# heiheishuang/MuDG

Hardware: AMD Instinct MI355X
Metric: DDIM denoise steps/sec, MDM1024 576x1024x16f (CFG: 2 UNet forwards + fused update per step, per clip) (higher is better)
Workload: dtype bf16; 1 GPU; MDM1024 latents (B=1,4,16,72,128) + c_concat 8ch, context (B,333,1024), 50-step uniform_trailing DDIM schedule, cfg 7.5, guidance_rescale 0.7, eta 1.0, v-prediction, dynamic rescale; clips_per_gpu=1, parallelism=clip-DP x1 (no in-step collective), launch=hipGraph replay of each UNet pass (cond+uncond batched)

## Files before the change

### mudg_amd/csrc/attention.hip

```cpp
#include "common.h"
#include <cstdlib>
#include <type_traits>

namespace {

constexpr int QB = 128;
constexpr int KB = 64;
constexpr int ALD = 72;
constexpr int ATILE = 64 * ALD;

template <bool TWO>
__global__ __launch_bounds__(256, 2) void attn_kernel(const MudgAttnDesc p, const int nqt, const int total) {
    __shared__ __attribute__((aligned(16))) h16 Ks[2 * ATILE];
    __shared__ __attribute__((aligned(16))) h16 Vs[2 * ATILE];

    const int tid = threadIdx.x, lane = tid & 63, wave = tid >> 6;
    const int l31 = lane & 31, hi = lane >> 5;

    int w;
    {
        const int q8 = total >> 3, r8 = total & 7;
        const int xcd = blockIdx.x & 7, idx = blockIdx.x >> 3;
        w = (xcd < r8 ? xcd * (q8 + 1) : r8 * (q8 + 1) + (xcd - r8) * q8) + idx;
    }
// ... 394 lines not shown
    u32x4 kr[2], vr[2];
    auto load_tiles = [&](int kt) {
        const int j0 = kt * KB;
#pragma unroll
        for (int i = 0; i < 2; ++i) {
            const int row = lrow + 32 * i;
            const int j = j0 + row;
            kr[i] = (j < p.Nk) ? ld16(Kp + (int64_t)j * p.ldk + kc * 8) : zero16();
            const int jc = j0 + kc * 8;
            u32x4 v = zero16();
            if (jc < p.Nk) {
                v = ld16(Vp + (int64_t)row * p.ldvt + jc);
                if (jc + 8 > p.Nk) {
                    h16x8 hv = as_h16x8(v);
#pragma unroll
                    for (int e = 0; e < 8; ++e) if (jc + e >= p.Nk) hv[e] = (h16)0.f;
                    v = as_u32x4(hv);
                }
            }
            vr[i] = v;
        }
    };
    const int vlo = (kc >> 1) * 16 + ((kc & 1) ? 4 : 0), vhi = (kc >> 1) * 16 + ((kc & 1) ? 12 : 8);
    auto stage = [&](int buf) {
#pragma unroll
        for (int i = 0; i < 2; ++i) {
            st16(&Ks[buf * ATILE + (lrow + 32 * i) * ALD + kc * 8], kr[i]);
            h16* vrow = &Vs[buf * ATILE + (lrow + 32 * i) * ALD];
            *reinterpret_cast<u32x2*>(vrow + vlo) = u32x2{vr[i][0], vr[i][1]};
            *reinterpret_cast<u32x2*>(vrow + vhi) = u32x2{vr[i][2], vr[i][3]};
        }
    };

    f32x16 o[2][2];
#pragma unroll
    for (int qb = 0; qb < 2; ++qb)
#pragma unroll
        for (int r = 0; r < 16; ++r) { o[qb][0][r] = 0.f; o[qb][1][r] = 0.f; }
    float m_run[2] = {-INFINITY, -INFINITY}, l_run[2] = {0.f, 0.f};
    const float c = p.q_prescaled ? 1.0f : p.scale * 1.4426950408889634f;

    const int nkt = (p.Nk + KB - 1) / KB;
    load_tiles(0);
    stage(0);
    __syncthreads();

    for (int kt = 0; kt < nkt; ++kt) {
        const int cur = kt & 1;
        const bool more = kt + 1 < nkt;
        if (more) load_tiles(kt + 1);

        f32x16 s[2][2];
#pragma unroll
        for (int sub = 0; sub < 2; ++sub) {
#pragma unroll
            for (int qb = 0; qb < 2; ++qb)
#pragma unroll
                for (int r = 0; r < 16; ++r) s[qb][sub][r] = 0.f;
            const h16* kp = Ks + cur * ATILE + (sub * 32 + l31) * ALD + hi * 8;
#pragma unroll
            for (int ks = 0; ks < 4; ++ks) {
                const h16x8 kf = *reinterpret_cast<const h16x8*>(kp + ks * 16);
                s[0][sub] = MFMA_32x32x16(kf, qf[0][ks], s[0][sub]);
                s[1][sub] = MFMA_32x32x16(kf, qf[1][ks], s[1][sub]);
            }
        }
        if (kt * KB + KB > p.Nk) {
#pragma unroll
            for (int sub = 0; sub < 2; ++sub)
#pragma unroll
                for (int r = 0; r < 16; ++r) {
                    const int j = kt * KB + sub * 32 + (r & 3) + 8 * (r >> 2) + 4 * hi;
                    if (j >= p.Nk) { s[0][sub][r] = -INFINITY; s[1][sub][r] = -INFINITY; }
                }
        }

        h16x8 pk[2][2][2];
#pragma unroll
        for (int qb = 0; qb < 2; ++qb) {
            float mx = s[qb][0][0];
#pragma unroll
            for (int r = 1; r < 16; ++r) mx = fmaxf(mx, s[qb][0][r]);
#pragma unroll
            for (int r = 0; r < 16; ++r) mx = fmaxf(mx, s[qb][1][r]);
            mx = fmaxf(mx, __shfl_xor(mx, 32, 64));
            const bool grew = !__all(mx <= m_run[qb]);
            const float m_new = grew ? fmaxf(m_run[qb], mx) : m_run[qb];
            const float alpha = grew ? __builtin_amdgcn_exp2f((m_run[qb] - m_new) * c) : 1.0f;
            const float mc = m_new * c;
            m_run[qb] = m_new;
            float ps = 0.f;
#pragma unroll
            for (int sub = 0; sub < 2; ++sub)
#pragma unroll
                for (int r = 0; r < 16; ++r) {
                    const float e = __builtin_amdgcn_exp2f(fmaf(s[qb][sub][r], c, -mc));
                    ps += e;
                    pk[qb][sub][r >> 3][r & 7] = (h16)e;
                }
            l_run[qb] = l_run[qb] * alpha + ps;
            if (grew) {
#pragma unroll
                for (int r = 0; r < 16; ++r) { o[qb][0][r] *= alpha; o[qb][1][r] *= alpha; }
            }
        }

#pragma unroll
        for (int dt = 0; dt < 2; ++dt) {
            const h16* vp = Vs + cur * ATILE + (dt * 32 + l31) * ALD + 8 * hi;
#pragma unroll
            for (int sub = 0; sub < 2; ++sub)
#pragma unroll
                for (int jj = 0; jj < 2; ++jj) {
                    const h16x8 vf = *reinterpret_cast<const h16x8*>(vp + sub * 32 + jj * 16);
                    o[0][dt] = MFMA_32x32x16(vf, pk[0][sub][jj], o[0][dt]);
                    o[1][dt] = MFMA_32x32x16(vf, pk[1][sub][jj], o[1][dt]);
                }
        }

        if (more) stage(cur ^ 1);
        __syncthreads();
    }

#pragma unroll
    for (int qb = 0; qb < 2; ++qb) {
        const float l_tot = l_run[qb] + __shfl_xor(l_run[qb], 32, 64);
        const float inv = 1.f / l_tot;
        if (p.Lse && qok[qb] && hi == 0) p.Lse[((int64_t)f * p.Nq + qrow[qb]) * p.heads + h] = m_run[qb] * c + __log2f(l_tot);
        if (qok[qb]) {
            h16* orow = Op + (int64_t)qrow[qb] * p.ldo;
#pragma unroll
            for (int dt = 0; dt < 2; ++dt)
#pragma unroll
                for (int g = 0; g < 4; ++g) {
                    h16* dst = orow + dt * 32 + 8 * g + 4 * hi;
                    float v[4];
#pragma unroll
                    for (int j = 0; j < 4; ++j) v[j] = o[qb][dt][4 * g + j] * inv;
                    if (p.accumulate) {
                        Pack8 old; old.u = *reinterpret_cast<const u32x2*>(dst);
#pragma unroll
                        for (int j = 0; j < 4; ++j) v[j] += (float)old.h[j];
                    }
                    Pack8 nw;
#pragma unroll
                    for (int j = 0; j < 4; ++j) nw.h[j] = (h16)v[j];
                    *reinterpret_cast<u32x2*>(dst) = nw.u;
                }
        }
    }
}

constexpr int DTILE = 64 * 64;
#ifdef MUDG_OPERAND_FP16
constexpr float LEAN_LIMIT = 32768.f;
#else
constexpr float LEAN_LIMIT = 1099511627776.f;
#endif

__device__ __forceinline__ __amdgpu_buffer_rsrc_t attn_rsrc(const h16* base) {
    return __builtin_amdgcn_make_buffer_rsrc(const_cast<h16*>(base), 0, (int)0x80000000u, 0x00020000);
}
typedef __attribute__((address_space(3))) void* attn_lptr_t;

typedef __attribute__((ext_vector_type(8))) int i32x8;

template <bool LEAN, bool F8>
__global__ __launch_bounds__(256, 2) void attn64d_kernel(const MudgAttnDesc p, const int nqt, const int total) {
    static_assert(LEAN || !F8, "the fp8 score path builds on the lean softmax");
    __shared__ __attribute__((aligned(1024))) h16 Ks[F8 ? DTILE : 2 * DTILE];
    __shared__ __attribute__((aligned(1024))) h16 Vs[2 * DTILE];

    const int tid = threadIdx.x, lane = tid & 63;
    const int wave = __builtin_amdgcn_readfirstlane(tid >> 6);
    const int l31 = lane & 31, hi = lane >> 5;
    int w;
    {
        const int q8 = total >> 3, r8 = total & 7;
        const int xcd = blockIdx.x & 7, idx = blockIdx.x >> 3;
        w = (xcd < r8 ? xcd * (q8 + 1) : r8 * (q8 + 1) + (xcd - r8) * q8) + idx;
    }
    const int pair = w / nqt, qt = w - pair * nqt;
    const int f = pair / p.heads, h = pair - f * p.heads;
    const int kvb = f / p.kv_div;

    const h16* Qp = reinterpret_cast<const h16*>(p.Q) + (int64_t)f * p.Nq * p.ldq + h * 64;
    const h16* Kp = reinterpret_cast<const h16*>(p.K) + (int64_t)kvb * p.Nk * p.ldk + h * 64;
    const h16* Vp = reinterpret_cast<const h16*>(p.Vt) + (int64_t)kvb * p.svt + (int64_t)(h * 64) * p.ldvt;
    h16* Op = reinterpret_cast<h16*>(p.O) + (int64_t)f * p.Nq * p.ldo + h * 64;

    int qrow[2];
    bool qok[2];
    h16x8 qf[2][F8 ? 1 : 4];
    i32x8 qf8[2];
    int qsc[2] = {127, 127};
    const unsigned char* K8p = nullptr;
    const unsigned char* Ksp = nullptr;
#pragma unroll
    for (int qb = 0; qb < 2; ++qb) {
        qrow[qb] = qt * 256 + wave * 64 + qb * 32 + l31;
        qok[qb] = qrow[qb] < p.Nq;
        if constexpr (F8) {
            const unsigned char* q8 = reinterpret_cast<const unsigned char*>(p.Q8) + ((int64_t)f * p.Nq + qrow[qb]) * p.ldq8 + h * 64 + hi * 16;
            const u32x4 a = qok[qb] ? ld16(q8) : zero16(), b = qok[qb] ? ld16(q8 + 32) : zero16();
            qf8[qb] = i32x8{(int)a[0], (int)a[1], (int)a[2], (int)a[3], (int)b[0], (int)b[1], (int)b[2], (int)b[3]};
            if (qok[qb]) qsc[qb] = reinterpret_cast<const unsigned char*>(p.Qs)[((int64_t)f * p.Nq + qrow[qb]) * p.ldqs + h * 2 + hi];
        } else {
#pragma unroll
            for (int ks = 0; ks < 4; ++ks)
                qf[qb][ks] = as_h16x8(qok[qb] ? ld16(Qp + (int64_t)qrow[qb] * p.ldq + ks * 16 + hi * 8) : zero16());
        }
    }
    if constexpr (F8) {
        K8p = reinterpret_cast<const unsigned char*>(p.K8) + (int64_t)kvb * p.Nk * p.ldk8 + h * 64;
        Ksp = reinterpret_cast<const unsigned char*>(p.Ks) + (int64_t)kvb * p.Nk * p.ldks + h * 2;
    }

    const __amdgpu_buffer_rsrc_t rK = F8 ? __builtin_amdgcn_make_buffer_rsrc(const_cast<unsigned char*>(K8p), 0, (int)0x80000000u, 0x00020000)
                                         : attn_rsrc(Kp);
    const __amdgpu_buffer_rsrc_t rV = attn_rsrc(Vp);
    unsigned vk[2], vv[2];
#pragma unroll
    for (int i = 0; i < 2; ++i) {
        const int row = 16 * wave + 8 * i + (lane >> 3), slot = lane & 7;
        const int chunk = slot ^ ((row >> 1) & 7);
        const int i16 = row & 15;
        const int key = (row & ~15) | (i16 & 3) | ((i16 & 8) >> 1) | ((i16 & 4) << 1);
        vk[i] = (unsigned)key * (unsigned)p.ldk * 2u + (unsigned)chunk * 16u;
        vv[i] = (unsigned)row * (unsigned)p.ldvt * 2u + (unsigned)chunk * 16u;
    }
    int kscale_off[2] = {0, 0};
    if constexpr (F8) {
        const int row = 16 * wave + (lane >> 2), slot = lane & 3;
        const int chunk = slot ^ ((row >> 2) & 3);
        const int i16 = row & 15;
        const int key = (row & ~15) | (i16 & 3) | ((i16 & 8) >> 1) | ((i16 & 4) << 1);
        vk[0] = (unsigned)key * (unsigned)p.ldk8 + (unsigned)chunk * 16u;
#pragma unroll
        for (int sub = 0; sub < 2; ++sub) {
            const int r = sub * 32 + l31, j16 = r & 15;
            const int k = (r & ~15) | (j16 & 3) | ((j16 & 8) >> 1) | ((j16 & 4) << 1);
            kscale_off[sub] = k * p.ldks + hi;
        }
    }
    auto request = [&](int kt, int buf) {
        const int sv = kt * 128;
        if constexpr (F8) {
            unsigned char* ks8 = reinterpret_cast<unsigned char*>(Ks);
            __builtin_amdgcn_raw_ptr_buffer_load_lds(rK, (attn_lptr_t)(ks8 + buf * 4096 + (16 * wave) * 64), 16, (int)vk[0], kt * 64 * p.ldk8, 0, 0);
        }
#pragma unroll
        for (int i = 0; i < 2; ++i) {
            if constexpr (!F8)
                __builtin_amdgcn_raw_ptr_buffer_load_lds(rK, (attn_lptr_t)(Ks + buf * DTILE + (16 * wave + 8 * i) * 64), 16, (int)vk[i], kt * 64 * p.ldk * 2, 0, 0);
            __builtin_amdgcn_raw_ptr_buffer_load_lds(rV, (attn_lptr_t)(Vs + buf * DTILE + (16 * wave + 8 * i) * 64), 16, (int)vv[i], sv, 0, 0);
        }
    };
    const int sw = (l31 >> 1) & 7;
    const int sw8 = (l31 >> 2) & 3;
    auto score_block = [&](int buf, int sub, f32x16& s0, f32x16& s1, int kscale) {
        if constexpr (F8) {
            const unsigned char* kp = reinterpret_cast<const unsigned char*>(Ks) + buf * 4096 + (sub * 32 + l31) * 64;
            const u32x4 a = ld16(kp + ((hi ^ sw8) << 4)), b = ld16(kp + (((2 + hi) ^ sw8) << 4));
            const i32x8 kf = {(int)a[0], (int)a[1], (int)a[2], (int)a[3], (int)b[0], (int)b[1], (int)b[2], (int)b[3]};
            s0 = __builtin_amdgcn_mfma_scale_f32_32x32x64_f8f6f4(kf, qf8[0], s0, 0, 0, 0, kscale, 0, qsc[0]);
            s1 = __builtin_amdgcn_mfma_scale_f32_32x32x64_f8f6f4(kf, qf8[1], s1, 0, 0, 0, kscale, 0, qsc[1]);
        } else {
            const h16* kp = Ks + buf * DTILE + (sub * 32 + l31) * 64;
#pragma unroll
            for (int ks = 0; ks < 4; ++ks) {
                const h16x8 kf = *reinterpret_cast<const h16x8*>(kp + (((ks * 2 + hi) ^ sw) << 3));
                s0 = MFMA_32x32x16(kf, qf[0][ks], s0);
                s1 = MFMA_32x32x16(kf, qf[1][ks], s1);
            }
        }
    };

    f32x16 o[2][2];
    float m_run[2], l_run[2];
    const float c = p.q_prescaled ? 1.0f : p.scale * 1.4426950408889634f;
    const int nkt = p.Nk / KB;
    bool overflow = false;

    auto key_loop = [&](auto lean_tag) {
        constexpr bool LN = decltype(lean_tag)::value;
#pragma unroll
        for (int qb = 0; qb < 2; ++qb) {
#pragma unroll
            for (int r = 0; r < 16; ++r) { o[qb][0][r] = 0.f; o[qb][1][r] = 0.f; }
            m_run[qb] = LN ? 0.f : -INFINITY;
            l_run[qb] = 0.f;
        }
        request(0, 0);
        __syncthreads();
        if constexpr (LN) {
            f32x16 s0[2][2];
#pragma unroll
            for (int sub = 0; sub < 2; ++sub) {
#pragma unroll
                for (int qb = 0; qb < 2; ++qb)
#pragma unroll
                    for (int r = 0; r < 16; ++r) s0[qb][sub][r] = 0.f;
                score_block(0, sub, s0[0][sub], s0[1][sub], F8 ? (int)Ksp[kscale_off[sub]] : 127);
            }
#pragma unroll
            for (int qb = 0; qb < 2; ++qb) {
                float mx = s0[qb][0][0];
#pragma unroll
                for (int r = 1; r < 16; ++r) mx = fmaxf(mx, s0[qb][0][r]);
#pragma unroll
                for (int r = 0; r < 16; ++r) mx = fmaxf(mx, s0[qb][1][r]);
                m_run[qb] = fmaxf(mx, __shfl_xor(mx, 32, 64));
            }
        }

        int ksc[2] = {127, 127};
        if constexpr (F8) { ksc[0] = Ksp[kscale_off[0]]; ksc[1] = Ksp[kscale_off[1]]; }
        for (int kt = 0; kt < nkt; ++kt) {
            const int cur = kt & 1;
            if (kt + 1 < nkt) request(kt + 1, cur ^ 1);
            int ksn[2] = {127, 127};
            if constexpr (F8) {
                if (kt + 1 < nkt) {
                    ksn[0] = Ksp[(int64_t)(kt + 1) * 64 * p.ldks + kscale_off[0]];
                    ksn[1] = Ksp[(int64_t)(kt + 1) * 64 * p.ldks + kscale_off[1]];
                }
            }

            f32x16 s[2][2];
#pragma unroll
            for (int sub = 0; sub < 2; ++sub) {
#pragma unroll
                for (int qb = 0; qb < 2; ++qb) {
                    const float init = LN ? -m_run[qb] : 0.f;
#pragma unroll
                    for (int r = 0; r < 16; ++r) s[qb][sub][r] = init;
                }
                score_block(cur, sub, s[0][sub], s[1][sub], ksc[sub]);
            }
            if constexpr (F8) { ksc[0] = ksn[0]; ksc[1] = ksn[1]; }

            h16x8 pk[2][2][2];
#pragma unroll
            for (int qb = 0; qb < 2; ++qb) {
                if constexpr (LN) {
                    float ps = 0.f;
#pragma unroll
                    for (int sub = 0; sub < 2; ++sub)
#pragma unroll
                        for (int r = 0; r < 16; ++r) {
                            const float e = __builtin_amdgcn_exp2f(s[qb][sub][r]);
                            ps += e;
                            pk[qb][sub][r >> 3][r & 7] = (h16)e;
                        }
                    l_run[qb] += ps;
                    overflow = overflow || !(ps <= LEAN_LIMIT);
                } else {
                    float mx = s[qb][0][0];
#pragma unroll
                    for (int r = 1; r < 16; ++r) mx = fmaxf(mx, s[qb][0][r]);
#pragma unroll
                    for (int r = 0; r < 16; ++r) mx = fmaxf(mx, s[qb][1][r]);
                    mx = fmaxf(mx, __shfl_xor(mx, 32, 64));
                    const bool grew = !__all(mx <= m_run[qb]);
                    const float m_new = grew ? fmaxf(m_run[qb], mx) : m_run[qb];
                    const float alpha = grew ? __builtin_amdgcn_exp2f((m_run[qb] - m_new) * c) : 1.0f;
                    const float mc = m_new * c;
                    m_run[qb] = m_new;
                    float ps = 0.f;
#pragma unroll
                    for (int sub = 0; sub < 2; ++sub)
#pragma unroll
                        for (int r = 0; r < 16; ++r) {
                            const float e = __builtin_amdgcn_exp2f(fmaf(s[qb][sub][r], c, -mc));
                            ps += e;
                            pk[qb][sub][r >> 3][r & 7] = (h16)e;
                        }
                    l_run[qb] = l_run[qb] * alpha + ps;
                    if (grew) {
#pragma unroll
                        for (int r = 0; r < 16; ++r) { o[qb][0][r] *= alpha; o[qb][1][r] *= alpha; }
                    }
                }
            }

#pragma unroll
            for (int dt = 0; dt < 2; ++dt) {
                const h16* vp = Vs + cur * DTILE + (dt * 32 + l31) * 64;
#pragma unroll
                for (int sub = 0; sub < 2; ++sub)
#pragma unroll
                    for (int jj = 0; jj < 2; ++jj) {
                        const h16x8 vf = *reinterpret_cast<const h16x8*>(vp + (((4 * sub + 2 * jj + hi) ^ sw) << 3));
                        o[0][dt] = MFMA_32x32x16(vf, pk[0][sub][jj], o[0][dt]);
                        o[1][dt] = MFMA_32x32x16(vf, pk[1][sub][jj], o[1][dt]);
                    }
            }
            __syncthreads();
        }
    };

    if constexpr (LEAN) {
        key_loop(std::true_type{});
        if (__syncthreads_or(overflow ? 1 : 0)) key_loop(std::false_type{});
    } else {
        key_loop(std::false_type{});
    }

#pragma unroll
    for (int qb = 0; qb < 2; ++qb) {
        const float l_tot = l_run[qb] + __shfl_xor(l_run[qb], 32, 64);
        const float inv = 1.f / l_tot;
        if (p.Lse && qok[qb] && hi == 0) p.Lse[((int64_t)f * p.Nq + qrow[qb]) * p.heads + h] = m_run[qb] * c + __log2f(l_tot);
        if (qok[qb]) {
            h16* orow = Op + (int64_t)qrow[qb] * p.ldo;
#pragma unroll
            for (int dt = 0; dt < 2; ++dt)
#pragma unroll
                for (int g = 0; g < 4; ++g) {
                    h16* dst = orow + dt * 32 + 8 * g + 4 * hi;
                    float v[4];
#pragma unroll
                    for (int j = 0; j < 4; ++j) v[j] = o[qb][dt][4 * g + j] * inv;
                    if (p.accumulate) {
                        Pack8 old; old.u = *reinterpret_cast<const u32x2*>(dst);
#pragma unroll
                        for (int j = 0; j < 4; ++j) v[j] += (float)old.h[j];
                    }
                    Pack8 nw;
#pragma unroll
                    for (int j = 0; j < 4; ++j) nw.h[j] = (h16)v[j];
                    *reinterpret_cast<u32x2*>(dst) = nw.u;
                }
        }
    }
}

constexpr int TATTN_ITEMS = 4;

template <int TP>
__global__ __launch_bounds__(256, TP == 16 ? 3 : 1) void tattn_kernel(const h16* __restrict__ QKV, h16* __restrict__ O,
                                                     int B, int T, int HW, int heads, int ldqkv, int ldo,
                                                     float scale, int total) {
    constexpr int DP = 64 / TP, DW = 64 / DP;
    __shared__ __attribute__((aligned(16))) h16 Ks[4][TP * 64];
    __shared__ __attribute__((aligned(16))) h16 Vs[4][TP * 64];

    const int tid = threadIdx.x, lane = tid & 63, wave = tid >> 6;
    const int tq = lane / DP, dp = lane % DP;
    const int C = heads * 64;
    const int w0 = (blockIdx.x * 4 + wave) * TATTN_ITEMS;

    u32x4 qn[DW / 8], kn[DW / 8], vn[DW / 8];
    int64_t rown = 0; int hn = 0; bool okn = false;
    auto fetch = [&](int w) {
        okn = w < total && tq < T;
        const int bp = w < total ? w / heads : 0;
        hn = w < total ? w - bp * heads : 0;
        const int b = bp / HW, px = bp - b * HW;
        rown = ((int64_t)(b * T + tq) * HW + px);
        const h16* src = QKV + rown * ldqkv + hn * 64 + dp * DW;
#pragma unroll
        for (int i = 0; i < DW / 8; ++i) {
            qn[i] = okn ? ld16(src + i * 8) : zero16();
            kn[i] = okn ? ld16(src + C + i * 8) : zero16();
            vn[i] = okn ? ld16(src + 2 * C + i * 8) : zero16();
        }
    };
    fetch(w0);

    for (int it = 0; it < TATTN_ITEMS; ++it) {
        if (w0 + it >= total) break;
        h16x8 qv[DW / 8];
        const int64_t row = rown; const int h = hn; const bool rok = okn;
        __builtin_amdgcn_wave_barrier();
#pragma unroll
        for (int i = 0; i < DW / 8; ++i) {
            qv[i] = as_h16x8(qn[i]);
            st16(&Ks[wave][tq * 64 + dp * DW + i * 8], kn[i]);
            st16(&Vs[wave][tq * 64 + dp * DW + i * 8], vn[i]);
        }
        __builtin_amdgcn_wave_barrier();
        if (it + 1 < TATTN_ITEMS) fetch(w0 + it + 1);

        float sc[TP];
        float mx = -INFINITY;
#pragma unroll
        for (int j = 0; j < TP; ++j) {
            float a = 0.f;
#pragma unroll
            for (int i = 0; i < DW / 8; ++i) {
                const h16x8 kk = *reinterpret_cast<const h16x8*>(&Ks[wave][j * 64 + dp * DW + i * 8]);
#pragma unroll
                for (int e = 0; e < 8; e += 2) {
                    const h16x2 qp = {qv[i][e], qv[i][e + 1]}, kp = {kk[e], kk[e + 1]};
                    a = DOT2_H16(qp, kp, a);
                }
            }
#pragma unroll
            for (int o = 1; o < DP; o <<= 1) a += __shfl_xor(a, o, 64);
            a = (j < T) ? a * scale : -INFINITY;
            sc[j] = a;
            mx = fmaxf(mx, a);
        }
        float sum = 0.f;
#pragma unroll
        for (int j = 0; j < TP; ++j) { sc[j] = __expf(sc[j] - mx); sum += sc[j]; }
        const float inv = 1.f / sum;

        float ov[DW];
#pragma unroll
        for (int d = 0; d < DW; ++d) ov[d] = 0.f;
#pragma unroll
        for (int j = 0; j < TP; ++j) {
            const float pj = sc[j] * inv;
#pragma unroll
            for (int i = 0; i < DW / 8; ++i) {
                const h16x8 vv = *reinterpret_cast<const h16x8*>(&Vs[wave][j * 64 + dp * DW + i * 8]);
#pragma unroll
                for (int e = 0; e < 8; ++e) ov[i * 8 + e] = fmaf(pj, (float)vv[e], ov[i * 8 + e]);
            }
        }
        if (rok) {
            h16* dst = O + row * ldo + h * 64 + dp * DW;
#pragma unroll
            for (int i = 0; i < DW / 8; ++i) {
                h16x8 t;
#pragma unroll
                for (int e = 0; e < 8; ++e) t[e] = (h16)ov[i * 8 + e];
                st16(dst + i * 8, as_u32x4(t));
            }
        }
    }
}


#if MUDG_PLANES == 1
#ifdef MUDG_OPERAND_FP16
typedef __attribute__((ext_vector_type(4))) _Float16 mf4;
#define MFMA_16x16x32(a, b, c) __builtin_amdgcn_mfma_f32_16x16x32_f16(a, b, c, 0, 0, 0)
#define MFMA_16x16x16(a, b, c) __builtin_amdgcn_mfma_f32_16x16x16f16(a, b, c, 0, 0, 0)
#else
typedef __attribute__((ext_vector_type(4))) short mf4;
#define MFMA_16x16x32(a, b, c) __builtin_amdgcn_mfma_f32_16x16x32_bf16(a, b, c, 0, 0, 0)
#define MFMA_16x16x16(a, b, c) __builtin_amdgcn_mfma_f32_16x16x16bf16_1k(a, b, c, 0, 0, 0)
#endif

__global__ __launch_bounds__(256) void tattn_mfma_kernel(const h16* __restrict__ QKV, h16* __restrict__ O,
                                                          int B, int T, int HW, int heads, int ldqkv, int ldo,
                                                          float scale, int total) {
    __shared__ __attribute__((aligned(16))) h16 Ts[4][3][16 * 64];
    const int tid = threadIdx.x, lane = tid & 63, wave = tid >> 6;
    const int c = lane & 15, g = lane >> 4;
    const int lr = lane >> 3, lj = lane & 7;
    const int C = heads * 64;
// ... 605 lines not shown
        const int b = bp / HW, px = bp - b * HW;
        pixn = (int64_t)b * T * HW + px;
#pragma unroll
        for (int s = 0; s < 2; ++s) {
            const int t = lr + 8 * s;
            const bool ok = item && t < T;
            const h16* src = QKV + (pixn + (int64_t)(ok ? t : 0) * HW) * ldqkv + hn * 64 + lj * 8;
#pragma unroll
            for (int x = 0; x < 3; ++x)
#pragma unroll
                for (int pc = 0; pc < 2; ++pc) nx[x][pc][s] = ok ? ld16(src + x * C + pc * ps) : zero16();
        }
    };
    fetch(w0);

    for (int it = 0; it < TATTN_SPLIT_ITEMS; ++it) {
        if (w0 + it >= total) break;
        const int64_t pix = pixn; const int h = hn;
        __builtin_amdgcn_wave_barrier();
#pragma unroll
        for (int s = 0; s < 2; ++s) {
            const int r = lr + 8 * s, z = fz(r >> 2);
#pragma unroll
            for (int pc = 0; pc < 2; ++pc) {
                st16(tile(0, pc) + r * 128 + ((lj ^ (r & 7)) << 4), nx[0][pc][s]);
                st16(tile(1, pc) + r * 128 + ((lj ^ (r & 7)) << 4), nx[1][pc][s]);
                u32x2 lo = {nx[2][pc][s][0], nx[2][pc][s][1]}, hi = {nx[2][pc][s][2], nx[2][pc][s][3]};
                *reinterpret_cast<u32x2*>(tile(2, pc) + r * 128 + (((2 * lj) ^ z) << 3)) = lo;
                *reinterpret_cast<u32x2*>(tile(2, pc) + r * 128 + (((2 * lj + 1) ^ z) << 3)) = hi;
            }
        }
        __builtin_amdgcn_wave_barrier();
        if (it + 1 < TATTN_SPLIT_ITEMS) fetch(w0 + it + 1);

        f32x4 st = {0.f, 0.f, 0.f, 0.f};
#pragma unroll
        for (int term = 0; term < 3; ++term) {
            const int kp = term == 1 ? 1 : 0, qp = term == 0 ? 1 : 0;
#pragma unroll
            for (int s = 0; s < 2; ++s) {
                const int off = c * 128 + (((g + 4 * s) ^ (c & 7)) << 4);
                st = __builtin_amdgcn_mfma_f32_16x16x32_bf16(as_h16x8(ld16(tile(1, kp) + off)), as_h16x8(ld16(tile(0, qp) + off)), st, 0, 0, 0);
            }
        }
        float sc[4];
        float mx = -INFINITY;
#pragma unroll
        for (int i = 0; i < 4; ++i) { sc[i] = (4 * g + i < T) ? st[i] * scale : -INFINITY; mx = fmaxf(mx, sc[i]); }
        mx = fmaxf(mx, __shfl_xor(mx, 16, 64));
        mx = fmaxf(mx, __shfl_xor(mx, 32, 64));
        float sum = 0.f;
        union { mf4s m; h16 e[4]; } p0, p1;
#pragma unroll
        for (int i = 0; i < 4; ++i) {
            const float pv = expf(sc[i] - mx);
            sum += pv;
            p0.e[i] = (h16)pv;
            p1.e[i] = (h16)(pv - (float)p0.e[i]);
        }
        sum += __shfl_xor(sum, 16, 64);
        sum += __shfl_xor(sum, 32, 64);

        float ov[16];
#pragma unroll
        for (int m = 0; m < 4; ++m) {
            union { mf4s m4; unsigned short e[4]; } v0, v1;
            const int u = (8 * (m >> 1) + 2 * (c >> 2) + (m & 1)) ^ fz(g);
#pragma unroll
            for (int j = 0; j < 4; ++j) {
                const int off = (4 * g + j) * 128 + (u << 3) + 2 * (c & 3);
                v0.e[j] = *reinterpret_cast<const unsigned short*>(tile(2, 0) + off);
                v1.e[j] = *reinterpret_cast<const unsigned short*>(tile(2, 1) + off);
            }
            f32x4 acc = {0.f, 0.f, 0.f, 0.f};
            acc = __builtin_amdgcn_mfma_f32_16x16x16bf16_1k(v0.m4, p1.m, acc, 0, 0, 0);
            acc = __builtin_amdgcn_mfma_f32_16x16x16bf16_1k(v1.m4, p0.m, acc, 0, 0, 0);
            acc = __builtin_amdgcn_mfma_f32_16x16x16bf16_1k(v0.m4, p0.m, acc, 0, 0, 0);
#pragma unroll
            for (int i = 0; i < 4; ++i) ov[4 * m + i] = acc[i] / sum;
        }
        if (c < T) {
            h16* dst = O + (pix + (int64_t)c * HW) * ldo + h * 64 + g * 8;
#pragma unroll
            for (int half = 0; half < 2; ++half) {
                float o8[8];
#pragma unroll
                for (int e = 0; e < 8; ++e) o8[e] = ov[half * 8 + e];
                store8_operand(dst + half * 32, ldo / PLANES, o8);
            }
        }
    }
}
#endif
#endif

}

extern "C" int mudg_attention(const MudgAttnDesc* dp, void* stream) {
    MUDG_REQUIRE(dp, "mudg_attention: null descriptor");
    const MudgAttnDesc d = *dp;
    MUDG_REQUIRE(d.Q && d.K && d.Vt && d.O, "mudg_attention: null pointer");
    MUDG_REQUIRE(d.F > 0 && d.heads > 0 && d.Nq > 0 && d.Nk > 0, "mudg_attention: empty problem");
    MUDG_REQUIRE(d.kv_div >= 1 && d.F % d.kv_div == 0, "mudg_attention: kv_div=%d F=%d", d.kv_div, d.F);
    MUDG_REQUIRE(d.ldq % (8 * PLANES) == 0 && d.ldk % (8 * PLANES) == 0 && d.ldvt % (8 * PLANES) == 0 && d.ldo % (4 * PLANES) == 0 &&
                 (d.svt & 7) == 0, "mudg_attention: row strides must be multiples of %d (ldo of %d)", 8 * PLANES, 4 * PLANES);
    MUDG_REQUIRE(d.ldvt / PLANES >= d.Nk, "mudg_attention: ldvt=%d < %d x Nk=%d", d.ldvt, PLANES, d.Nk);
    MUDG_REQUIRE(d.ldq / PLANES >= d.heads * 64 && d.ldk / PLANES >= d.heads * 64 && d.ldo / PLANES >= d.heads * 64,
                 "mudg_attention: row strides too small for %d heads", d.heads);
    MUDG_REQUIRE(aligned16(d.Q) && aligned16(d.K) && aligned16(d.Vt) && aligned16(d.O), "mudg_attention: alignment");
    if (d.K2) {
        MUDG_REQUIRE(d.Vt2 && d.Nk2 > 0 && d.kv_div2 >= 1 && d.F % d.kv_div2 == 0, "mudg_attention: second key/value set");
        MUDG_REQUIRE(d.ldk2 % (8 * PLANES) == 0 && d.ldvt2 % (8 * PLANES) == 0 && (d.svt2 & 7) == 0 && d.ldvt2 / PLANES >= d.Nk2 &&
                     d.ldk2 / PLANES >= d.heads * 64 && aligned16(d.K2) && aligned16(d.Vt2), "mudg_attention: second key/value set strides");
        MUDG_REQUIRE(!d.accumulate, "mudg_attention: accumulate and a second key/value set are exclusive");
    }
    MUDG_REQUIRE(!d.Lse || (PLANES == 1 && !d.K2 && !d.q_prescaled && !d.Q8 && !d.accumulate),
                 "mudg_attention: Lse (the softmax statistics for mudg_attention_bwd) comes from the plain single-set kernels of the 16-bit builds");
    const int nqt = (d.Nq + QB - 1) / QB;
    const int64_t total = (int64_t)nqt * d.F * d.heads;
    MUDG_REQUIRE(total < (1ll << 31), "mudg_attention: grid too large");
    hipStream_t s = reinterpret_cast<hipStream_t>(stream);
    const int slot = mudg_prof_begin(MUDG_FAM_ATTN, s);
    static int var = -1;
    if (var < 0) var = mudg_variant("ATTN_Q", 0);
    const bool wide = !d.K2 && (var == 64 ? d.Nq >= 256 : (var == 32 ? false : (d.Nq >= 512 && d.Nk >= 256)));
#if MUDG_PLANES > 1
    {
        constexpr int smem = 4 * PLANES * ATILE * (int)sizeof(h16);
        if (const int rc = mudg_lds_opt_in<&attn_split_kernel<false>>(smem, "mudg_attention")) return rc;
        if (const int rc = mudg_lds_opt_in<&attn_split_kernel<true>>(smem, "mudg_attention")) return rc;
        bool dma_ok = false;
#if MUDG_PLANES == 2
        dma_ok = wide && d.Nk % 64 == 0 && (int64_t)d.Nk * d.ldk * 2 < (1ll << 31) && (int64_t)64 * d.ldvt * 2 + (int64_t)d.Nk * 2 + d.ldvt < (1ll << 31);
        if (dma_ok) {
            if (const int rc = mudg_lds_opt_in<&attn_split_dma_kernel<true>>(SPLIT_DMA_SMEM, "mudg_attention")) return rc;
            if (const int rc = mudg_lds_opt_in<&attn_split_dma_kernel<false>>(SPLIT_DMA_SMEM, "mudg_attention")) return rc;
            if (d.q_prescaled) hipLaunchKernelGGL(attn_split_dma_kernel<true>, dim3((unsigned)total), dim3(256), SPLIT_DMA_SMEM, s, d, nqt, (int)total);
            else hipLaunchKernelGGL(attn_split_dma_kernel<false>, dim3((unsigned)total), dim3(256), SPLIT_DMA_SMEM, s, d, nqt, (int)total);
        }
#endif
        (void)wide;
        if (dma_ok) {}
        else if (d.K2) hipLaunchKernelGGL(attn_split_kernel<true>, dim3((unsigned)total), dim3(256), smem, s, d, nqt, (int)total);
        else hipLaunchKernelGGL(attn_split_kernel<false>, dim3((unsigned)total), dim3(256), smem, s, d, nqt, (int)total);
    }
#else
    MUDG_REQUIRE(!d.Q8 || wide, "mudg_attention: the MX-fp8 score path serves the long self-attention kernel only (Nq >= 512, Nk >= 256)");
    if (wide) {
        const int nqt2 = (d.Nq + 255) / 256;
        const int64_t total2 = (int64_t)nqt2 * d.F * d.heads;
        static int dma = -1, lean = -1;
        if (dma < 0) dma = mudg_variant("ATTN_DMA", 1);
        if (lean < 0) lean = mudg_variant("ATTN_LEAN", 1);
        const bool dma_ok = dma && d.Nk % 64 == 0 && (int64_t)d.Nk * d.ldk * 2 < (1ll << 31) && (int64_t)64 * d.ldvt * 2 + (int64_t)d.Nk * 2 < (1ll << 31);
        if (d.Q8) {
            MUDG_REQUIRE(dma_ok && d.q_prescaled && d.K8 && d.Qs && d.Ks && !d.accumulate, "mudg_attention: the MX-fp8 score path needs "
                         "q_prescaled, Nk %% 64 == 0 and all four of Q8 / K8 / Qs / Ks");
            MUDG_REQUIRE((d.ldq8 & 15) == 0 && (d.ldk8 & 15) == 0 && aligned16(d.Q8) && aligned16(d.K8) && d.ldq8 >= d.heads * 64 &&
                         d.ldk8 >= d.heads * 64 && d.ldqs >= d.heads * 2 && d.ldks >= d.heads * 2 && (int64_t)d.Nk * d.ldk8 < (1ll << 31),
                         "mudg_attention: fp8 strides");
            hipLaunchKernelGGL((attn64d_kernel<true, true>), dim3((unsigned)total2), dim3(256), 0, s, d, nqt2, (int)total2);
        }
        else if (dma_ok && d.q_prescaled && lean) hipLaunchKernelGGL((attn64d_kernel<true, false>), dim3((unsigned)total2), dim3(256), 0, s, d, nqt2, (int)total2);
        else if (dma_ok) hipLaunchKernelGGL((attn64d_kernel<false, false>), dim3((unsigned)total2), dim3(256), 0, s, d, nqt2, (int)total2);
        else hipLaunchKernelGGL(attn64q_kernel, dim3((unsigned)total2), dim3(256), 0, s, d, nqt2, (int)total2);
    } else {
        static int xv = -1;
        if (xv < 0) xv = mudg_variant("ATTN_X", 1);
        int xq = (int)(total / 1024);
        xq = xq > 8 ? 8 : xq;
        if (xv && xq >= 2 && d.Nk <= 2 * KB && (!d.K2 || d.Nk2 <= KB)) {
            constexpr int smem = 2 * XK_TILES * ATILE * (int)sizeof(h16);
            if (const int rc = mudg_lds_opt_in<&xattn_kernel<false>>(smem, "mudg_attention")) return rc;
            if (const int rc = mudg_lds_opt_in<&xattn_kernel<true>>(smem, "mudg_attention")) return rc;
            const int nqc = (nqt + xq - 1) / xq;
            const int64_t totx = (int64_t)nqc * d.F * d.heads;
            if (d.K2) hipLaunchKernelGGL(xattn_kernel<true>, dim3((unsigned)totx), dim3(256), smem, s, d, nqt, xq, nqc, (int)totx);
            else hipLaunchKernelGGL(xattn_kernel<false>, dim3((unsigned)totx), dim3(256), smem, s, d, nqt, xq, nqc, (int)totx);
        }
        else if (d.K2) hipLaunchKernelGGL(attn_kernel<true>, dim3((unsigned)total), dim3(256), 0, s, d, nqt, (int)total);
        else hipLaunchKernelGGL(attn_kernel<false>, dim3((unsigned)total), dim3(256), 0, s, d, nqt, (int)total);
    }
#endif
    const int rc = mudg_check_launch("mudg_attention");
    const double bh = (double)d.F * d.heads;
    mudg_prof_end(slot, s, 4.0 * bh * d.Nq * (double)(d.Nk + (d.K2 ? d.Nk2 : 0)) * 64.0,
                  bh * (2.0 * d.Nq + 2.0 * d.Nk / d.kv_div + (d.K2 ? 2.0 * d.Nk2 / d.kv_div2 : 0.0)) * 64.0 * 2.0);
    return rc;
}

#if MUDG_PLANES == 1
namespace {
__global__ __launch_bounds__(256) void quantize_mxfp8_kernel(const h16* __restrict__ X, int ldx, int64_t rows, int nblk,
                                                              unsigned char* __restrict__ Y, int ldy, unsigned char* __restrict__ S, int lds) {
    const int64_t i = (int64_t)blockIdx.x * 256 + threadIdx.x;
    if (i >= rows * nblk) return;
    const int64_t r = i / nblk;
    const int b = (int)(i - r * nblk);
    const h16* src = X + r * ldx + b * 32;
    float v[32];
    float amax = 0.f;
#pragma unroll
    for (int q = 0; q < 4; ++q) {
        const h16x8 t = as_h16x8(ld16(src + q * 8));
#pragma unroll
        for (int e = 0; e < 8; ++e) { v[q * 8 + e] = (float)t[e]; amax = fmaxf(amax, fabsf(v[q * 8 + e])); }
    }
    const int E = mx_block_exponent(amax);
    const float inv = __uint_as_float((unsigned)(127 - E) << 23);
    u32x4 lo, hi4;
#pragma unroll
    for (int q = 0; q < 8; ++q) {
        const unsigned w = mx_pack4_e4m3(v[q * 4], v[q * 4 + 1], v[q * 4 + 2], v[q * 4 + 3], inv);
        if (q < 4) lo[q] = w; else hi4[q - 4] = w;
    }
    unsigned char* dst = Y + r * ldy + b * 32;
    st16(dst, lo);
    st16(dst + 16, hi4);
    S[r * lds + b] = (unsigned char)(E + 127);
}
}
#endif

extern "C" int mudg_quantize_mxfp8(const void* X, int ldx, int64_t rows, int cols, void* Y8, int ldy, void* S, int lds, void* stream) {
#if MUDG_PLANES == 1
    MUDG_REQUIRE(X && Y8 && S && rows > 0 && cols > 0 && cols % 32 == 0, "mudg_quantize_mxfp8: bad arguments");
    MUDG_REQUIRE((ldx & 7) == 0 && (ldy & 15) == 0 && ldx >= cols && ldy >= cols && lds >= cols / 32 && aligned16(X) && aligned16(Y8),
                 "mudg_quantize_mxfp8: strides / alignment");
    hipStream_t s = reinterpret_cast<hipStream_t>(stream);
    const int nblk = cols / 32;
    const int64_t n = rows * nblk;
    const int slot = mudg_prof_begin(MUDG_FAM_MISC, s);
    hipLaunchKernelGGL(quantize_mxfp8_kernel, dim3((unsigned)((n + 255) / 256)), dim3(256), 0, s, (const h16*)X, ldx, rows, nblk,
                       (unsigned char*)Y8, ldy, (unsigned char*)S, lds);
    const int rc = mudg_check_launch("mudg_quantize_mxfp8");
    mudg_prof_end(slot, s, 0.0, (double)rows * cols * 3.0);
    return rc;
#else
    (void)X; (void)ldx; (void)rows; (void)cols; (void)Y8; (void)ldy; (void)S; (void)lds; (void)stream;
    MUDG_FAIL(MUDG_EUNSUPPORTED, "mudg_quantize_mxfp8: fp8 scores belong to the 16-bit operand builds");
#endif
}

extern "C" int mudg_temporal_attention(const void* QKV, void* O, int B, int T, int HW, int heads,
                                       int ldqkv, int ldo, float scale, void* stream) {
    MUDG_REQUIRE(QKV && O, "mudg_temporal_attention: null pointer");
    MUDG_REQUIRE(B > 0 && HW > 0 && heads > 0, "mudg_temporal_attention: empty problem");
    MUDG_REQUIRE(T >= 1 && T <= 32, "mudg_temporal_attention: T=%d outside [1,32]", T);
    MUDG_REQUIRE(ldqkv % (8 * PLANES) == 0 && ldo % (8 * PLANES) == 0 && aligned16(QKV) && aligned16(O), "mudg_temporal_attention: alignment");
    MUDG_REQUIRE(ldqkv / PLANES >= 3 * heads * 64 && ldo / PLANES >= heads * 64, "mudg_temporal_attention: row strides too small");
    const int64_t total = (int64_t)B * HW * heads;
    MUDG_REQUIRE(total < (1ll << 31), "mudg_temporal_attention: grid too large");
    hipStream_t s = reinterpret_cast<hipStream_t>(stream);
    const int slot = mudg_prof_begin(MUDG_FAM_TATTN, s);
#if MUDG_PLANES > 1
    const unsigned grid = (unsigned)((total + 3) / 4);
#if MUDG_PLANES == 2
    static int use_mfma = -1;
    if (use_mfma < 0) use_mfma = mudg_variant("TATTN_MFMA", 1);
    if (T <= 16 && use_mfma)
        hipLaunchKernelGGL(tattn_split_mfma_kernel, dim3((unsigned)((total + 4 * TATTN_SPLIT_ITEMS - 1) / (4 * TATTN_SPLIT_ITEMS))), dim3(256), 0, s,
                           (const h16*)QKV, (h16*)O, B, T, HW, heads, ldqkv, ldo, scale, (int)total);
    else
#endif
    if (T <= 16)
        hipLaunchKernelGGL(tattn_split_kernel<16>, dim3(grid), dim3(256), 0, s, (const h16*)QKV, (h16*)O, B, T, HW, heads,
                           ldqkv, ldo, scale, (int)total);
    else
        hipLaunchKernelGGL(tattn_split_kernel<32>, dim3(grid), dim3(256), 0, s, (const h16*)QKV, (h16*)O, B, T, HW, heads,
                           ldqkv, ldo, scale, (int)total);
#else
    const unsigned grid = (unsigned)((total + 4 * TATTN_ITEMS - 1) / (4 * TATTN_ITEMS));
    static int use_mfma = -1;
    if (use_mfma < 0) use_mfma = mudg_variant("TATTN_MFMA", 1);
    if (T <= 16 && use_mfma)
        hipLaunchKernelGGL(tattn_mfma_kernel, dim3(grid), dim3(256), 0, s, (const h16*)QKV, (h16*)O, B, T, HW, heads,
                           ldqkv, ldo, scale, (int)total);
    else if (T <= 16)
        hipLaunchKernelGGL(tattn_kernel<16>, dim3(grid), dim3(256), 0, s, (const h16*)QKV, (h16*)O, B, T, HW, heads,
                           ldqkv, ldo, scale, (int)total);
    else
        hipLaunchKernelGGL(tattn_kernel<32>, dim3(grid), dim3(256), 0, s, (const h16*)QKV, (h16*)O, B, T, HW, heads,
                           ldqkv, ldo, scale, (int)total);
#endif
    const int rc = mudg_check_launch("mudg_temporal_attention");
    mudg_prof_end(slot, s, 4.0 * total * (double)T * T * 64.0, (double)total * T * 64.0 * 2.0 * 4.0);
    return rc;
}
```

Measured before the change: 8.400 steps/s.

## Triple-buffer K/V tiles in the long self-attention kernel with fine-grained waitcnt

Moves the 64-dim DMA attention kernel from double to triple buffering of K/V tiles in LDS. Tile kt+2 is prefetched while kt is computed, and the full __syncthreads is replaced by a partial vmcnt wait plus a raw s_barrier, so loads stay in flight across iterations. The fp8 key scales are now fetched through buffer loads, and the lean-overflow vote goes through a shared LDS flag instead of __syncthreads_or. This adds LDS use per block, which may lower occupancy. It also relies on the vmcnt count matching the number of DMA instructions issued per tile.

```diff
diff --git a/mudg_amd/csrc/attention.hip b/mudg_amd/csrc/attention.hip
--- a/mudg_amd/csrc/attention.hip
+++ b/mudg_amd/csrc/attention.hip
@@ -570,6 +570,7 @@
 }
 
 constexpr int DTILE = 64 * 64;
+constexpr int DSLOTS = 3;
 #ifdef MUDG_OPERAND_FP16
 constexpr float LEAN_LIMIT = 32768.f;
 #else
@@ -583,11 +584,25 @@
 
 typedef __attribute__((ext_vector_type(8))) int i32x8;
 
-template <bool LEAN, bool F8>
+template <bool LEAN, bool F8, bool PIPE>
 __global__ __launch_bounds__(256, 2) void attn64d_kernel(const MudgAttnDesc p, const int nqt, const int total) {
     static_assert(LEAN || !F8, "the fp8 score path builds on the lean softmax");
-    __shared__ __attribute__((aligned(1024))) h16 Ks[F8 ? DTILE : 2 * DTILE];
-    __shared__ __attribute__((aligned(1024))) h16 Vs[2 * DTILE];
+    constexpr int KSLOT = F8 ? DTILE / 2 : DTILE;
+    constexpr int NDMA = F8 ? 3 : 4;
+    h16* Ks;
+    h16* Vs;
+    int* ovf = nullptr;
+    if constexpr (PIPE) {
+        __shared__ __attribute__((aligned(1024))) h16 lds[DSLOTS * (KSLOT + DTILE) + 8];
+        Ks = lds;
+        Vs = lds + DSLOTS * KSLOT;
+        ovf = reinterpret_cast<int*>(lds + DSLOTS * (KSLOT + DTILE));
+    } else {
+        __shared__ __attribute__((aligned(1024))) h16 Ks2[2 * KSLOT];
+        __shared__ __attribute__((aligned(1024))) h16 Vs2[2 * DTILE];
+        Ks = Ks2;
+        Vs = Vs2;
+    }
 
     const int tid = threadIdx.x, lane = tid & 63;
     const int wave = __builtin_amdgcn_readfirstlane(tid >> 6);
@@ -661,16 +676,20 @@
             kscale_off[sub] = k * p.ldks + hi;
         }
     }
+    const __amdgpu_buffer_rsrc_t rKs = F8 ? __builtin_amdgcn_make_buffer_rsrc(const_cast<unsigned char*>(Ksp), 0, (int)0x80000000u, 0x00020000) : rV;
+    auto kscale = [&](int kt, int sub) -> int {
+        return __builtin_amdgcn_raw_buffer_load_b8(rKs, kscale_off[sub], kt * 64 * p.ldks, 0);
+    };
     auto request = [&](int kt, int buf) {
         const int sv = kt * 128;
         if constexpr (F8) {
             unsigned char* ks8 = reinterpret_cast<unsigned char*>(Ks);
-            __builtin_amdgcn_raw_ptr_buffer_load_lds(rK, (attn_lptr_t)(ks8 + buf * 4096 + (16 * wave) * 64), 16, (int)vk[0], kt * 64 * p.ldk8, 0, 0);
+            __builtin_amdgcn_raw_ptr_buffer_load_lds(rK, (attn_lptr_t)(ks8 + buf * (2 * KSLOT) + (16 * wave) * 64), 16, (int)vk[0], kt * 64 * p.ldk8, 0, 0);
         }
 #pragma unroll
         for (int i = 0; i < 2; ++i) {
             if constexpr (!F8)
-                __builtin_amdgcn_raw_ptr_buffer_load_lds(rK, (attn_lptr_t)(Ks + buf * DTILE + (16 * wave + 8 * i) * 64), 16, (int)vk[i], kt * 64 * p.ldk * 2, 0, 0);
+                __builtin_amdgcn_raw_ptr_buffer_load_lds(rK, (attn_lptr_t)(Ks + buf * KSLOT + (16 * wave + 8 * i) * 64), 16, (int)vk[i], kt * 64 * p.ldk * 2, 0, 0);
             __builtin_amdgcn_raw_ptr_buffer_load_lds(rV, (attn_lptr_t)(Vs + buf * DTILE + (16 * wave + 8 * i) * 64), 16, (int)vv[i], sv, 0, 0);
         }
     };
@@ -678,13 +697,13 @@
     const int sw8 = (l31 >> 2) & 3;
     auto score_block = [&](int buf, int sub, f32x16& s0, f32x16& s1, int kscale) {
         if constexpr (F8) {
-            const unsigned char* kp = reinterpret_cast<const unsigned char*>(Ks) + buf * 4096 + (sub * 32 + l31) * 64;
+            const unsigned char* kp = reinterpret_cast<const unsigned char*>(Ks) + buf * (2 * KSLOT) + (sub * 32 + l31) * 64;
             const u32x4 a = ld16(kp + ((hi ^ sw8) << 4)), b = ld16(kp + (((2 + hi) ^ sw8) << 4));
             const i32x8 kf = {(int)a[0], (int)a[1], (int)a[2], (int)a[3], (int)b[0], (int)b[1], (int)b[2], (int)b[3]};
             s0 = __builtin_amdgcn_mfma_scale_f32_32x32x64_f8f6f4(kf, qf8[0], s0, 0, 0, 0, kscale, 0, qsc[0]);
             s1 = __builtin_amdgcn_mfma_scale_f32_32x32x64_f8f6f4(kf, qf8[1], s1, 0, 0, 0, kscale, 0, qsc[1]);
         } else {
-            const h16* kp = Ks + buf * DTILE + (sub * 32 + l31) * 64;
+            const h16* kp = Ks + buf * KSLOT + (sub * 32 + l31) * 64;
 #pragma unroll
             for (int ks = 0; ks < 4; ++ks) {
                 const h16x8 kf = *reinterpret_cast<const h16x8*>(kp + (((ks * 2 + hi) ^ sw) << 3));
@@ -709,8 +728,17 @@
             m_run[qb] = LN ? 0.f : -INFINITY;
             l_run[qb] = 0.f;
         }
-        request(0, 0);
-        __syncthreads();
+        int ksc[2] = {127, 127};
+        if constexpr (F8) { ksc[0] = kscale(0, 0); ksc[1] = kscale(0, 1); }
+        if constexpr (PIPE) {
+            request(0, 0);
+            request(nkt > 1 ? 1 : 0, 1);
+            asm volatile("s_waitcnt vmcnt(%0) lgkmcnt(0)" :: "n"(NDMA) : "memory");
+            __builtin_amdgcn_s_barrier();
+        } else {
+            request(0, 0);
+            __syncthreads();
+        }
         if constexpr (LN) {
             f32x16 s0[2][2];
 #pragma unroll
@@ -719,7 +747,7 @@
                 for (int qb = 0; qb < 2; ++qb)
 #pragma unroll
                     for (int r = 0; r < 16; ++r) s0[qb][sub][r] = 0.f;
-                score_block(0, sub, s0[0][sub], s0[1][sub], F8 ? (int)Ksp[kscale_off[sub]] : 127);
+                score_block(0, sub, s0[0][sub], s0[1][sub], ksc[sub]);
             }
 #pragma unroll
             for (int qb = 0; qb < 2; ++qb) {
@@ -732,18 +760,20 @@
             }
         }
 
-        int ksc[2] = {127, 127};
-        if constexpr (F8) { ksc[0] = Ksp[kscale_off[0]]; ksc[1] = Ksp[kscale_off[1]]; }
+        int cur = 0, nxt = 2;
         for (int kt = 0; kt < nkt; ++kt) {
-            const int cur = kt & 1;
-            if (kt + 1 < nkt) request(kt + 1, cur ^ 1);
+            if constexpr (!PIPE) {
+                cur = kt & 1;
+                if (kt + 1 < nkt) request(kt + 1, cur ^ 1);
+            }
             int ksn[2] = {127, 127};
             if constexpr (F8) {
                 if (kt + 1 < nkt) {
-                    ksn[0] = Ksp[(int64_t)(kt + 1) * 64 * p.ldks + kscale_off[0]];
-                    ksn[1] = Ksp[(int64_t)(kt + 1) * 64 * p.ldks + kscale_off[1]];
-                }
-            }
+                    ksn[0] = kscale(kt + 1, 0);
+                    ksn[1] = kscale(kt + 1, 1);
+                }
+            }
+            if constexpr (PIPE) request(kt + 2 < nkt ? kt + 2 : nkt - 1, nxt);
 
             f32x16 s[2][2];
 #pragma unroll
@@ -814,11 +844,26 @@
                         o[1][dt] = MFMA_32x32x16(vf, pk[1][sub][jj], o[1][dt]);
                     }
             }
-            __syncthreads();
-        }
+            if constexpr (PIPE) {
+                asm volatile("s_waitcnt vmcnt(%0) lgkmcnt(0)" :: "n"(NDMA) : "memory");
+                __builtin_amdgcn_s_barrier();
+                cur = cur == DSLOTS - 1 ? 0 : cur + 1;
+                nxt = nxt == DSLOTS - 1 ? 0 : nxt + 1;
+            } else {
+                __syncthreads();
+            }
+        }
+        if constexpr (PIPE) asm volatile("s_waitcnt vmcnt(0)" ::: "memory");
     };
 
-    if constexpr (LEAN) {
+    if constexpr (LEAN && PIPE) {
+        if (tid == 0) *ovf = 0;
+        key_loop(std::true_type{});
+        if (overflow) *ovf = 1;
+        asm volatile("s_waitcnt lgkmcnt(0)" ::: "memory");
+        __builtin_amdgcn_s_barrier();
+        if (*ovf) key_loop(std::false_type{});
+    } else if constexpr (LEAN) {
         key_loop(std::true_type{});
         if (__syncthreads_or(overflow ? 1 : 0)) key_loop(std::false_type{});
     } else {
@@ -1730,6 +1775,13 @@
         static int dma = -1, lean = -1;
         if (dma < 0) dma = mudg_variant("ATTN_DMA", 1);
         if (lean < 0) lean = mudg_variant("ATTN_LEAN", 1);
+#ifdef MUDG_DEBUG_VARIANTS
+        static int pipe = -1;
+        if (pipe < 0) pipe = mudg_variant("ATTN_PIPE", 1);
+#define MUDG_ATTN64D(LN, F8) (pipe ? attn64d_kernel<LN, F8, true> : attn64d_kernel<LN, F8, false>)
+#else
+#define MUDG_ATTN64D(LN, F8) (attn64d_kernel<LN, F8, true>)
+#endif
         const bool dma_ok = dma && d.Nk % 64 == 0 && (int64_t)d.Nk * d.ldk * 2 < (1ll << 31) && (int64_t)64 * d.ldvt * 2 + (int64_t)d.Nk * 2 < (1ll << 31);
         if (d.Q8) {
             MUDG_REQUIRE(dma_ok && d.q_prescaled && d.K8 && d.Qs && d.Ks && !d.accumulate, "mudg_attention: the MX-fp8 score path needs "
@@ -1737,11 +1789,12 @@
             MUDG_REQUIRE((d.ldq8 & 15) == 0 && (d.ldk8 & 15) == 0 && aligned16(d.Q8) && aligned16(d.K8) && d.ldq8 >= d.heads * 64 &&
                          d.ldk8 >= d.heads * 64 && d.ldqs >= d.heads * 2 && d.ldks >= d.heads * 2 && (int64_t)d.Nk * d.ldk8 < (1ll << 31),
                          "mudg_attention: fp8 strides");
-            hipLaunchKernelGGL((attn64d_kernel<true, true>), dim3((unsigned)total2), dim3(256), 0, s, d, nqt2, (int)total2);
-        }
-        else if (dma_ok && d.q_prescaled && lean) hipLaunchKernelGGL((attn64d_kernel<true, false>), dim3((unsigned)total2), dim3(256), 0, s, d, nqt2, (int)total2);
-        else if (dma_ok) hipLaunchKernelGGL((attn64d_kernel<false, false>), dim3((unsigned)total2), dim3(256), 0, s, d, nqt2, (int)total2);
+            hipLaunchKernelGGL(MUDG_ATTN64D(true, true), dim3((unsigned)total2), dim3(256), 0, s, d, nqt2, (int)total2);
+        }
+        else if (dma_ok && d.q_prescaled && lean) hipLaunchKernelGGL(MUDG_ATTN64D(true, false), dim3((unsigned)total2), dim3(256), 0, s, d, nqt2, (int)total2);
+        else if (dma_ok) hipLaunchKernelGGL(MUDG_ATTN64D(false, false), dim3((unsigned)total2), dim3(256), 0, s, d, nqt2, (int)total2);
         else hipLaunchKernelGGL(attn64q_kernel, dim3((unsigned)total2), dim3(256), 0, s, d, nqt2, (int)total2);
+#undef MUDG_ATTN64D
     } else {
         static int xv = -1;
         if (xv < 0) xv = mudg_variant("ATTN_X", 1);
```

Measured after the change: 8.471 steps/s (median of 6 runs). No clear change (+0.8%).
